# victoriyaforsythe/PyRayHF

Measured on AMD Instinct MI355X. Metric: virtual-height integrals/s (profile x frequency pairs), higher is better.
Workload: dtype f64

## Files before the change

### include/prhf.h

```cpp
#ifndef PRHF_H
#define PRHF_H

#include <stdint.h>

#ifdef __cplusplus
extern "C" {
#endif

#define PRHF_ABI_VERSION 4

#define PRHF_OK        0
#define PRHF_EINVAL   -1
#define PRHF_ENEGDEN  -2
#define PRHF_EPEAK0   -3
#define PRHF_EHIP     -4
#define PRHF_ENOMEM   -5

#define PRHF_MODE_O 0
#define PRHF_MODE_X 1

#define PRHF_FLAG_DEVICE_PTRS 0x1u
#define PRHF_FLAG_ASYNC       0x2u
#define PRHF_FLAG_GRID_STABLE 0x4u
#define PRHF_FLAG_SHARED_FIELD 0x8u
// ... 242 lines not shown
                              const double* scan_elevation_deg, int64_t n_scan, double earth_radius_km, double s_max_km,
                              double rtol, double atol, double max_step_km, double z_ground_km, double top, double left,
                              double right, int32_t renormalize_every, double fill_n, double fill_grad, double fill_mup,
                              double elev_tol_deg, int32_t max_iter, int32_t n_hops, double* out, uint32_t flags);

int prhf_gradient_hop_skip_counters(prhf_ctx* ctx, uint64_t* counters);

int prhf_pair_plan_counters(prhf_ctx* ctx, uint64_t* counters);

int prhf_panel_counters(prhf_ctx* ctx, uint64_t* counters);

int prhf_panel_upper_counters(prhf_ctx* ctx, uint64_t* counters);

int prhf_panel_plan_counters(prhf_ctx* ctx, uint64_t* counters);

int prhf_stream_launches(prhf_ctx* ctx, uint64_t* count);

int prhf_occupancy(prhf_ctx* ctx, int64_t n_alt, int32_t math, int32_t* workgroups_per_cu);

int prhf_sync(prhf_ctx* ctx);

int prhf_last_kernel_ms(prhf_ctx* ctx, double* ms);

int prhf_recent_kernel_ms(prhf_ctx* ctx, double* ms, int32_t capacity, int32_t* n);

#ifdef __cplusplus
}
#endif
#endif
```

### pyrayhf_amd/_native.py

```python

from __future__ import annotations

import ctypes
import os
import threading

_HERE = os.path.dirname(os.path.abspath(__file__))
LIB_PATH = os.environ.get("PRHF_LIB") or os.path.join(_HERE, "libprhf.so")

OK, EINVAL, ENEGDEN, EPEAK0, EHIP, ENOMEM = 0, -1, -2, -3, -4, -5
MODE_O, MODE_X = 0, 1
FLAG_DEVICE_PTRS, FLAG_ASYNC, FLAG_GRID_STABLE, FLAG_SHARED_FIELD = 0x1, 0x2, 0x4, 0x8
MATH_FAITHFUL, MATH_FAST, MATH_AUTO = 0, 1, 2
ABI_VERSION = 4

c_double_p = ctypes.POINTER(ctypes.c_double)


class Segment(ctypes.Structure):
    _fields_ = [("prof_begin", ctypes.c_int64), ("prof_end", ctypes.c_int64),
                ("mode", ctypes.c_int32), ("n_points", ctypes.c_int32),
                ("mult_offset", ctypes.c_int64), ("out_offset", ctypes.c_int64)]


# ... 134 lines not shown
                                   [ctypes.c_int64] + [ctypes.c_void_p, ctypes.c_int64] + [ctypes.c_double] * 9 +
                                   [ctypes.c_int32] + [ctypes.c_double] * 4 +
                                   [ctypes.c_int32, ctypes.c_int32, ctypes.c_void_p, ctypes.c_uint32]),
    "prhf_gradient_hop_muf_f64": (ctypes.c_int, [ctypes.c_void_p, ctypes.c_int32] + [ctypes.c_void_p] * 3 +
                                  [ctypes.c_int64, ctypes.c_int64, ctypes.c_void_p, ctypes.c_void_p, ctypes.c_int32,
                                   ctypes.c_int32] + [ctypes.c_void_p] * 3 +
                                  [ctypes.c_int64, ctypes.c_double, ctypes.c_double, ctypes.c_int32, ctypes.c_void_p,
                                   ctypes.c_int64] + [ctypes.c_double] * 9 + [ctypes.c_int32] + [ctypes.c_double] * 4 +
                                  [ctypes.c_int32, ctypes.c_int32, ctypes.c_void_p, ctypes.c_uint32]),
    "prhf_gradient_skip_counters": (ctypes.c_int, [ctypes.c_void_p, ctypes.POINTER(ctypes.c_uint64)]),
    "prhf_gradient_hop_skip_counters": (ctypes.c_int, [ctypes.c_void_p, ctypes.POINTER(ctypes.c_uint64)]),
    "prhf_pair_plan_counters": (ctypes.c_int, [ctypes.c_void_p, ctypes.POINTER(ctypes.c_uint64)]),
    "prhf_panel_counters": (ctypes.c_int, [ctypes.c_void_p, ctypes.POINTER(ctypes.c_uint64)]),
    "prhf_panel_upper_counters": (ctypes.c_int, [ctypes.c_void_p, ctypes.POINTER(ctypes.c_uint64)]),
    "prhf_panel_plan_counters": (ctypes.c_int, [ctypes.c_void_p, ctypes.POINTER(ctypes.c_uint64)]),
    "prhf_stream_launches": (ctypes.c_int, [ctypes.c_void_p, ctypes.POINTER(ctypes.c_uint64)]),
    "prhf_occupancy": (ctypes.c_int, [ctypes.c_void_p, ctypes.c_int64, ctypes.c_int32,
                                      ctypes.POINTER(ctypes.c_int32)]),
    "prhf_sync": (ctypes.c_int, [ctypes.c_void_p]),
    "prhf_last_kernel_ms": (ctypes.c_int, [ctypes.c_void_p, ctypes.POINTER(ctypes.c_double)]),
    "prhf_recent_kernel_ms": (ctypes.c_int, [ctypes.c_void_p, ctypes.POINTER(ctypes.c_double), ctypes.c_int32,
                                             ctypes.POINTER(ctypes.c_int32)]),
}

_lib = None
_lib_lock = threading.Lock()


def load():
    global _lib
# ... 321 lines not shown
    def panel_counters(self):
        buf = (ctypes.c_uint64 * 2)()
        raise_for(self._lib.prhf_panel_counters(self._h, buf))
        return tuple(int(v) for v in buf)

    def panel_upper_counters(self):
        buf = (ctypes.c_uint64 * 2)()
        raise_for(self._lib.prhf_panel_upper_counters(self._h, buf))
        return tuple(int(v) for v in buf)

    def panel_plan_counters(self):
        buf = (ctypes.c_uint64 * 1)()
        raise_for(self._lib.prhf_panel_plan_counters(self._h, buf))
        return tuple(int(v) for v in buf)

    def stream_launches(self):
        n = ctypes.c_uint64(0)
        raise_for(self._lib.prhf_stream_launches(self._h, ctypes.byref(n)))
        return int(n.value)

    def occupancy(self, n_alt, math):
        n = ctypes.c_int32(0)
        raise_for(self._lib.prhf_occupancy(self._h, int(n_alt), int(math), ctypes.byref(n)))
        return n.value

    def sync(self):
        return self._lib.prhf_sync(self._h)

    def last_kernel_ms(self):
        ms = ctypes.c_double(0.0)
# ... 36 lines not shown
```

### pyrayhf_amd/csrc/prhf_api.cpp

```cpp

#include <hip/hip_runtime_api.h>

#include <algorithm>
#include <cctype>
#include <cmath>
#include <cstdarg>
#include <cstdio>
#include <cstdlib>
#include <cstring>
#include <new>
#include <string>
#include <vector>
#include <xmmintrin.h>

#include "prhf.h"
#include "prhf_kernels.h"
#include "prhf_plan.h"

namespace {

thread_local std::string g_err;

int fail(int code, const char* fmt, ...) {
    char buf[512];
// ... 880 lines not shown
        (e = create_events_untimed(c->slab_up, 3)) != hipSuccess ||
        (e = create_events_untimed(c->slab_done, 3)) != hipSuccess ||
        (e = create_events(c->ring0, prhf_ctx::kTimingRing)) != hipSuccess ||
        (e = create_events(c->ring1, prhf_ctx::kTimingRing)) != hipSuccess ||
        (e = hipMalloc(reinterpret_cast<void**>(&c->d_status), kStatusWords * sizeof(unsigned))) != hipSuccess ||
        (e = hipHostMalloc(reinterpret_cast<void**>(&c->h_status), PRHF_STATUS_WORDS * sizeof(unsigned),
                           hipHostMallocMapped | hipHostMallocCoherent)) != hipSuccess ||
        (e = hipHostGetDevicePointer(reinterpret_cast<void**>(&c->h_status_dev), c->h_status, 0)) != hipSuccess ||
        (e = hipMemset(c->d_status, 0, kStatusWords * sizeof(unsigned))) != hipSuccess ||
        (e = hipHostMalloc(reinterpret_cast<void**>(&c->h_pack), kPackBytes, hipHostMallocMapped | hipHostMallocCoherent)) !=
            hipSuccess ||
        (e = hipHostGetDevicePointer(reinterpret_cast<void**>(&c->h_pack_dev), c->h_pack, 0)) != hipSuccess ||
        (e = hipMalloc(reinterpret_cast<void**>(&c->d_words), 2 * sizeof(unsigned long long))) != hipSuccess ||
        (e = hipHostMalloc(reinterpret_cast<void**>(&c->h_words), 2 * sizeof(unsigned long long),
                           hipHostMallocDefault)) != hipSuccess ||
        (e = hipMalloc(reinterpret_cast<void**>(&c->d_plan_counters), 7 * sizeof(unsigned long long))) != hipSuccess ||
        (e = hipMemset(c->d_plan_counters, 0, 7 * sizeof(unsigned long long))) != hipSuccess ||
        (e = prhf::configure_kernels(staged_lds_bytes(kMaxAlt), kStreamLdsMax)) != hipSuccess) {
        prhf_ctx_destroy(c);
        return fail(PRHF_EHIP, "context setup failed: %s", hipGetErrorString(e));
    }
    c->stream = c->own_stream;
    std::memset(c->h_status, 0, PRHF_STATUS_WORDS * sizeof(unsigned));
#ifdef PRHF_DIAG
    for (const KnobName& k : kKnobNames) {
        std::string env = "PRHF_";
        for (const char* p = k.name; *p; ++p) env += (char)std::toupper((unsigned char)*p);
        if (const char* v = std::getenv(env.c_str())) c->knobs.*(k.field) = std::min(k.hi, std::max(k.lo, std::atof(v)));
    }
#endif
    (void)hipDeviceGetAttribute(&c->cu_count, hipDeviceAttributeMultiprocessorCount, device);
    if (hipDeviceGetAttribute(&c->large_bar, hipDeviceAttributeIsLargeBar, device) != hipSuccess) c->large_bar = 0;
// ... 1967 lines not shown
    counters[0] = w[0] - w[1];
    counters[1] = w[1];
    return PRHF_OK;
}

int prhf_panel_plan_counters(prhf_ctx* c, uint64_t* counters) {
    if (!c || !counters) return fail(PRHF_EINVAL, "null pointer");
    DeviceScope device_scope_(c->device);
    unsigned long long w[1] = {0};
    HIP_TRY(hipStreamSynchronize(c->stream));
    HIP_TRY(hipMemcpy(w, c->d_plan_counters + 6, sizeof w, hipMemcpyDeviceToHost));
    counters[0] = w[0];
    return PRHF_OK;
}

int prhf_stream_launches(prhf_ctx* c, uint64_t* count) {
    if (!c || !count) return fail(PRHF_EINVAL, "null pointer");
    *count = c->stream_launches;
    return PRHF_OK;
}

int prhf_occupancy(prhf_ctx* c, int64_t n_alt, int32_t math, int32_t* workgroups_per_cu) {
    if (!c || !workgroups_per_cu) return fail(PRHF_EINVAL, "null pointer");
    if (n_alt < 1 || n_alt > kMaxAlt) return fail(PRHF_EINVAL, "n_alt out of range");
    ENTER_DEVICE(c->device);
    int n = 0;
    HIP_TRY(prhf::query_occupancy(math, staged_lds_bytes(n_alt), &n));
    *workgroups_per_cu = n;
    return PRHF_OK;
}
// ... 47 lines not shown
```

### pyrayhf_amd/csrc/prhf_kernels.h

```cpp
#ifndef PRHF_KERNELS_H
#define PRHF_KERNELS_H

#include <hip/hip_runtime_api.h>
#include <stddef.h>
#include <stdint.h>

#define PRHF_KMODE_O 0
#define PRHF_KMODE_X 1

#define PRHF_STATUS_NEGDEN 0x1
#define PRHF_STATUS_PEAK0  0x2
#define PRHF_STATUS_BADINDEX 0x4
#define PRHF_STATUS_BADFIELD 0x20
#define PRHF_STATUS_PATHLEN 0x40
#define PRHF_STATUS_WORDS 8
#define PRHF_STATUS_NANINPUT 0x10
#define PRHF_STATUS_BADGROUP 0x8
#define PRHF_STATUS_STALL 0x80

#ifndef PRHF_BLOCK_THREADS
#define PRHF_BLOCK_THREADS 512
#endif
#ifndef PRHF_SHORT_THREADS
#define PRHF_SHORT_THREADS 512
// ... 66 lines not shown
    long long tail_prof;
    int tail_bpp;
    int panel_upper;
    double well_conditioned;
    int lean;
    int prio;
    long long sp_off;
    int strided_lower;
    int panel_lower;
    int panel_nodes;
    int strided_grade;
    int pair_plan;
    int thread_scan;
};

struct KArgs {
    const double* freq;
    const double* den;
    const double* bmag;
    const double* bpsi;
    const double* alt;
    const double* mult;
    const double* pairs;
    const double* ftab;
    double* out;
    double* partial;
    double* altmin;
    unsigned* status;
    unsigned* queue;
    long long n_blocks;
// ... 406 lines not shown
```

### pyrayhf_amd/csrc/prhf_kernels.hip

```cpp

#include <hip/hip_runtime.h>
#include <stdint.h>

#include "prhf_crmath.h"
#include "prhf_kernels.h"

namespace prhf {

namespace {

constexpr double kPlasma = 8.97866275;
constexpr double kGyro = 2.799249247e10;
constexpr double kBackoff = 1e-6;
constexpr double kDegToRad = 0.017453292519943295;
constexpr double kUnmagTol = 1e-12;
constexpr double kLightKmS = 299792.458;
constexpr double kPolyAngle = 3e-4;
constexpr double kQuadAngle = 4e-5;
constexpr double kTrigAngle = 0.05;
constexpr double kLinTol = 1e-10;

struct __attribute__((aligned(16))) Node {
    double alt, off, den, sden, b, sb, u0, u1, u2, u3, psi, spsi;
};
// ... 73 lines not shown
    const int hi = __builtin_amdgcn_update_dpp(__double2hiint(into_lane_0), __double2hiint(v), 0x138, 0xf, 0xf, false);
    return __hiloint2double(hi, lo);
}

__device__ __forceinline__ double uniform(double v) {
    const int lo = __builtin_amdgcn_readfirstlane(__double2loint(v));
    const int hi = __builtin_amdgcn_readfirstlane(__double2hiint(v));
    return __hiloint2double(hi, lo);
}
__device__ __forceinline__ int uniform(int v) { return __builtin_amdgcn_readfirstlane(v); }
constexpr int kStridedLowerBit = 1 << 30;
constexpr int kPanelLowerBit = 1 << 29;
constexpr int kPanelNodes4Bit = 1 << 28;
constexpr int kStridedGradeBit = 1 << 27;
constexpr int kPanelUpperBit = (int)(1u << 31);
constexpr int kPanelFar = 16;
constexpr int kPanelStateShift = 28;
#define PRHF_PANEL_NODES_DECL [[maybe_unused]] static __device__ const double kPanelNodes[8]
#define PRHF_PANEL_PAIRS_DECL static __device__ __attribute__((aligned(16))) const double kPanelPairs[(PRHF_PANEL_N_MAX + 1) * 16]
#include "prhf_panel_table.inc"
#define PRHF_PANEL4_PAIRS_DECL static __device__ __attribute__((aligned(16))) const double kPanel4Pairs[(PRHF_PANEL4_N_MAX + 1) * 8]
#include "prhf_panel4_table.inc"
static_assert(PRHF_PANEL4_N_MAX == PRHF_PANEL_N_MAX, "both tables end at the same piece length");
static_assert(PRHF_PANEL_BLOCK == 64 || PRHF_PANEL_BLOCK == 128, "the weight table ends at 128 points");
static_assert(PRHF_PANEL_BLOCK <= PRHF_PANEL_N_MAX, "a piece holds at most one block");
static_assert(PRHF_PANEL_MIN_SEGMENT >= 1 && (PRHF_PANEL_MIN_SEGMENT & (PRHF_PANEL_MIN_SEGMENT - 1)) == 0,
              "a power of two: the closed form squares its way up");

__device__ __forceinline__ double rsqrt_cubic(double x) {
    const double y = __builtin_amdgcn_rsq(x);
    const double t = x * y;
    const double e = __builtin_fma(-t, y, 1.0);
// ... 819 lines not shown
}
template <class MAt>
__device__ __forceinline__ int panel_first_point(int j, double rkj, double kj, double n1, int i_last, bool& ok, MAt m_at) {
#pragma clang fp contract(fast)
    const int guess = stretch_guess((double)j * rkj, n1);
    const int base = min(max(guess, 0) + 3, i_last) - 3;
    bool hit[4];
#pragma unroll
    for (int q = 0; q < 4; ++q) hit[q] = (int)(m_at(base + q) * kj) >= j;
    ok = j <= 0 || (guess == base && !hit[0] && hit[3]);
    return j <= 0 ? 0 : base + (hit[1] ? 1 : (hit[2] ? 2 : 3));
}
__device__ __forceinline__ int panel_region_end(int lo2) { return ((lo2 + 4) & ~63) & ~(PRHF_PANEL_BLOCK - 1); }
__device__ __forceinline__ int panel_upper_end(int lo0) { return (lo0 + 4) & ~63; }
__device__ __forceinline__ int panel_level(double m, double kj) { return (int)(m * kj); }

template <bool G>
__device__ __forceinline__ TopSegment top_segment(const NodeSpace<G>& nodes_v, int j, double span, double cY) {
#pragma clang fp contract(fast)
    const unsigned nd = __umul24((unsigned)j, (unsigned)sizeof(Node));
    const double o = nodes_v.f64(nd + 8), s = span;
    const double den = nodes_v.f64(nd + 16), sden = nodes_v.f64(nd + 24), b = nodes_v.f64(nd + 32), sb = nodes_v.f64(nd + 40),
                 u0 = nodes_v.f64(nd + 48), u1 = nodes_v.f64(nd + 56), u2 = nodes_v.f64(nd + 64), u3 = nodes_v.f64(nd + 72);
    TopSegment t;
    const SegLinear lin = seg_linear(o, den, sden, b, sb, s, cY);
    t.d0 = lin.d0;  t.d1 = lin.d1;
    t.b0 = lin.b0;  t.b1 = lin.b1;
    t.q0 = u0 + o * (u1 + o * (u2 + o * u3));
    t.q1 = s * (u1 + o * (2.0 * u2 + 3.0 * o * u3));
    t.q2 = (s * s) * (u2 + 3.0 * o * u3);
// ... 253 lines not shown
        }
    };
    constexpr bool STRIDED = TOP && MODE == PRHF_KMODE_X && !CHECK && !G;
    const int i_last_s = last_special;
    bool strided_on = false;
    bool lower_on = false;
    double sc1 = 0.0;
    sp_off = uniform(sp_off);
    const bool lower_req = (sp_off & kStridedLowerBit) != 0;
    const bool panel_req = (sp_off & kPanelLowerBit) != 0;
    const bool nodes4_req = (sp_off & kPanelNodes4Bit) != 0;
    constexpr bool grade_req = GRADE;
    static_assert(!UPPER || (STRIDED && !HINT), "only an instance with the panel block has the upper region");
    sp_off &= ~(kStridedLowerBit | kPanelLowerBit | kPanelNodes4Bit | kStridedGradeBit | kPanelUpperBit);
    constexpr int kUpperKept = 16, kUpperRegion = 8;
    int panel_state = 0;
    asm volatile("" : "+v"(panel_state));
    if (STRIDED && sp_off > 0 && n_seg > 0 && first == 0 && last_special >= 0 && end >= PRHF_TOP3_MIN_POINTS) {
        if constexpr (UPPER) {
            if (plan_panel) {
                typedef unsigned int u32x2 __attribute__((ext_vector_type(2)));
                const u32x2 vc = __builtin_amdgcn_raw_buffer_load_b64(rsrc, 0, sp_off * (int)sizeof(double2) + 8, 0);
                __builtin_memcpy(&sc1, &vc, sizeof sc1);
                strided_on = true;
                lower_on = lower_req;
            } else {
                const u32x4 vh = __builtin_amdgcn_raw_buffer_load_b128(rsrc, 0, sp_off * (int)sizeof(double2), 0);
                double2 gh;
                __builtin_memcpy(&gh, &vh, sizeof gh);
                const int hw = uniform((int)vh.x);
                strided_on = (hw & 1) == 0;
// ... 124 lines not shown
        int S_R = 0, E_R = 0, n_R = 0;
        const double n1 = (double)i_last_s, rkj = uniform(1.0 / kj);
        int j_b0 = seg_j[2];
        auto index_of = [&](double m) {
            const double A = __builtin_fma(1.0 - m, 22025.465794806718, 1.0);
            if (!(A > 0.0)) return 1e9;
            const double ln_a = (double)__builtin_amdgcn_logf((float)A) * 0.6931471805599453;
            return fmin(fmax(__builtin_fma(-ln_a, n1 * 0.1, n1), -1e9), 1e9);
        };
        auto x_of = [&](int j) { return index_of((double)j * rkj); };
        if (lower && panel_req && end < 65536) {
            bool panel_ok = false;
            int S_P = 0;
            constexpr int B = PRHF_PANEL_BLOCK, kLogB = B == 128 ? 7 : 6;
            const double c0 = 1.0 / 22025.465794806718;
            panel_state = 2;
            asm volatile("" : "+v"(panel_state));
            auto first_point = [&](int j, bool& ok) {
                return panel_first_point(j, rkj, kj, n1, i_last_s, ok, [&](int i) {
                    typedef unsigned int u32x2 __attribute__((ext_vector_type(2)));
                    const u32x2 v = __builtin_amdgcn_raw_buffer_load_b64(rsrc, (unsigned)i * (unsigned)sizeof(double2), 0, 0);
                    double mq;
                    __builtin_memcpy(&mq, &v, sizeof mq);
                    return mq;
                });
            };
            auto region_end = [&]() { return panel_region_end(seg_lo[2]); };
            constexpr bool REC = UPPER && PLANNABLE;
            unsigned pw3 = 0u, pw5 = 0u;
            if constexpr (REC) {
                const unsigned plan_s = (unsigned)uniform((int)plan_v);
// ... 42 lines not shown
                bool fail = false;
                int j_0 = j_s, left = j_e - j_s + 1;
                int j_e_lo = j_e, e_v = E_lo, s_v = S_P;
                if constexpr (UPPER) {
                    asm volatile("" : "+v"(j_e_lo), "+v"(s_v));
                    int up;
                    if (from_rec) {
                        up = (int)((pw3 >> 10) & 3u);
                    } else {
                        const u32x4 vu = __builtin_amdgcn_raw_buffer_load_b128(rsrc, 0, (upper_end() - 1) * (int)sizeof(double2), 0);
                        double2 gu;
                        __builtin_memcpy(&gu, &vu, sizeof gu);
                        up = uniform(panel_level(gu.x, kj)) - (seg_j[0] - 1);
                    }
                    if (up == 0 || up == 1) {
                        panel_state = 2 | kUpperRegion;
                        left = seg_j[0] + up - j_s;
                        e_v = upper_end();
                    } else {
                        panel_state = 2 | kUpperKept;
                    }
                    asm volatile("" : "+v"(e_v));
                }
#pragma unroll 1
                while (left > 0) {
                    int E_P = E_lo, S_L = S_P;
                    if constexpr (UPPER) {
                        asm volatile("" : "+v"(j_e_lo), "+v"(e_v), "+v"(s_v));
                        E_P = e_v;
                        S_L = s_v;
                    }
                    const bool live = lane < left;
                    const int j_g = live ? j_0 + lane : j_0;
                    bool ok;
                    const int fq = first_point(j_g, ok);
                    const int p = live ? max(fq, S_L) : E_P;
                    const int p_next = __shfl_down(p, 1);
                    const int n = live && lane < 63 ? max(min(p_next, E_P) - p, 0) : 0;
                    const int k = (n + B - 1) >> kLogB;
                    int L = n;
                    if (__any(k > 1)) {
                        int q = (int)((float)n * __builtin_amdgcn_rcpf((float)max(k, 1)));
                        q += q * k < n ? 1 : 0;
                        q -= (q - 1) * k >= n ? 1 : 0;
                        L = k > 1 ? q : n;
                    }
                    const unsigned nd = __umul24((unsigned)j_g, (unsigned)sizeof(Node));
                    const double o = nodes_v.f64(nd + 8), den = nodes_v.f64(nd + 16), sden = nodes_v.f64(nd + 24),
                                 bf = nodes_v.f64(nd + 32), sb = nodes_v.f64(nd + 40);
                    const double sl = cX * (sden * span) + r2 * (cYs * (sb * span));
                    const double gap = 1.0 - cX * (den + sden * o) - r2 * (cYs * (bf + sb * o));
                    const double m_hi = (double)(j_g + 1) * rkj;
                    const double g_lo = gap - sl * ((double)j_g * rkj), g_hi = gap - sl * m_hi;
                    const bool big = n > 8;
                    const bool levels = g_lo >= 1e-6 && g_hi >= 1e-6;
                    bool clear = levels;
                    const bool far = sl > 0.0 && (n1 * 0.1) * g_hi >= (double)(4 * B + 2) * (sl * ((1.0 - m_hi) + c0));
                    const int k_chk = big && clear && !far && __builtin_fabs(sl) > 1e-300 ? k : 0;
                    if (__any(k_chk > 0)) {
                        const double i_sing = index_of(gap / sl);
                        for (int i = 0; __ballot(i < k_chk) != 0ull; ++i) {
                            const int n_i = min(L, n - i * L);
                            const double c = (double)(p + i * L) + 0.5 * (double)(n_i - 1);
                            if (i < k_chk && n_i > 8)
                                clear = clear && __builtin_fabs(i_sing - c) >= fmax(32.0, 4.0 * (double)n_i);
                        }
                    }
                    int lvl = 0;
                    if (nodes4_req) {
                        bool open = n > 0;
                        for (int t = 0;; ++t) {
                            if (open) {
                                const int n_s = (L + (1 << t) - 1) >> t;
                                const double kk = (double)(kPanelFar * n_s + 2);
                                const double i_far = sl < 0.0 ? ((double)p + 0.5 * (double)((L >> t) - 1)) - kk
                                                              : ((double)(p + n - 1) - 0.5 * (double)(n_s - 1)) + kk;
                                const double e_far = (double)__builtin_amdgcn_exp2f((float)(i_far * (s10 * 1.4426950408889634)));
                                lvl = t;
                                open = !(n_s <= 4 || (levels && (1.0 + c0) * sl - gap <= sl * ((1.0 + c0) * e_far)));
                            }
                            if (__ballot(open) == 0ull) break;
                        }
                    }
                    const int cnt = n > 0 ? k << lvl : 0;
                    if constexpr (UPPER) {
                        int bad_v = (live && !ok) || (big && !clear) || cnt > 128 ? 1 : 0;
                        fail = __ballot(bad_v != 0) != 0ull;
                        if (fail) {
                            asm volatile("" : "+v"(bad_v));
                            if (!upper_now() || __ballot(bad_v != 0 && j_g < seg_j[0] - 3) != 0ull) break;
                            fail = false;
                            if (left <= 63) {
                                panel_state = 2 | kUpperKept;
                                e_v = region_end();
                                left = uniform(j_e_lo) - j_0 + 1;
                                continue;
                            }
                        }
                    } else {
                        fail = __ballot((live && !ok) || (big && !clear) || cnt > 128) != 0ull;
                        if (fail) break;
                    }
                    int total = min(63, left), n_take = total;
                    if constexpr (UPPER) {
                        if (left > 63 && upper_now()) total = n_take = min(total, seg_j[0] - 3 - j_0);
                    }
                    unsigned lst_a = n > 0 && (!UPPER || lane < total) ? (unsigned)p | ((unsigned)n << 16) : 0u, lst_b = 0u;
                    if (__ballot(cnt != (live && lane < 63 ? 1 : 0)) != 0ull) {
                        int incl = cnt;
                        incl += __builtin_amdgcn_update_dpp(0, incl, 0x111, 0xf, 0xf, false);
                        incl += __builtin_amdgcn_update_dpp(0, incl, 0x112, 0xf, 0xf, false);
                        incl += __builtin_amdgcn_update_dpp(0, incl, 0x114, 0xf, 0xf, false);
                        incl += __builtin_amdgcn_update_dpp(0, incl, 0x118, 0xf, 0xf, false);
                        incl += __builtin_amdgcn_update_dpp(0, incl, 0x142, 0xa, 0xf, false);
                        incl += __builtin_amdgcn_update_dpp(0, incl, 0x143, 0xc, 0xf, false);
                        n_take = __builtin_popcountll(__ballot((UPPER ? lane < total : live && lane < 63) && incl <= 128));
                        total = __builtin_amdgcn_readlane(incl, n_take - 1);
// ... 73 lines not shown
                                eval(eb);
                                break;
                            }
                            fetch(k0, ea);
                            eval(eb);
                        }
                    }
                }
                panel_ok = !fail;
                if constexpr (UPPER) S_P = uniform(s_v);
                if (!panel_ok) accm = 0.0;
                g0 = grid_at(first);
            }
            if constexpr (UPPER) {
                const int flags = uniform(panel_state);
                panel_state = !panel_ok ? 2 : ((flags & kUpperRegion) != 0 ? 3 : 4);
                asm volatile("" : "+v"(panel_state));
                if (panel_ok) {
                    S_R = S_P;
                    E_R = (flags & kUpperRegion) != 0 ? upper_end() : region_end();
                    n_R = -1;
                }
            } else if (panel_ok) {
                panel_state = 1;
                asm volatile("" : "+v"(panel_state));
                S_R = S_P;
                E_R = region_end();
                n_R = -1;
            }
        }
        if (lower && n_R >= 0) {
// ... 86 lines not shown
                    idx = (j_whole + (t0 + lane - 32 * n_R)) << 3;
                    coef = 8.0;
                }
                const u32x4 vm = __builtin_amdgcn_raw_buffer_load_b128(rsrc, (unsigned)idx * (unsigned)sizeof(double2), 0, 0);
                double2 gm;
                __builtin_memcpy(&gm, &vm, sizeof gm);
                gm.y = coef * (sc1 * ((1.0 - gm.x) + c0));
                accm = lean_step<MODE, false, POLY, HINT, G>(gm, span, a0v, kj, cX, hcY2, accm, wc, viol, nodes_v, cur);
            }
            }
            first = E_R;
            g0 = grid_at(first);
        }
    }
    if (TOP) {
        const int sidx_0 = UPPER && uniform(panel_state) == 3 ? 0 : n_seg - 1;
#pragma unroll 1
        for (int sidx = sidx_0; sidx >= 0 && !(CHECK && viol); --sidx) {
            const int lo_b = sidx == 0 ? seg_lo[0] : (sidx == 1 ? seg_lo[1] : seg_lo[2]);
            const int begin_s = (lo_b + 63) & ~63;
            const int end_s = sidx == 0 ? whole_end : ((sidx == 1 ? seg_lo[0] : seg_lo[1]) & ~63);
            const int j_s = seg_j[0] - sidx;
            run_indexed(begin_s);
            if (!(CHECK && viol)) {
                top = top_segment(nodes_v, j_s, span, cYs);
                if (STRIDED && strided_on) {
                    const int lo_s = sidx == 0 ? seg_lo[0] : (sidx == 1 ? seg_lo[1] : seg_lo[2]);
                    const int q_s = sidx == 0 ? i_last_s - 1 : (sidx == 1 ? seg_lo[0] - 1 : seg_lo[1] - 1);
                    strided_run(lo_s, q_s, begin_s, sidx);
                }
                run_top(end_s);
// ... 14 lines not shown
        } else {
            if (!live) g = make_double2(HINT ? uniform(g0.x) : 0.0, 0.0);
            a1 = lean_step<MODE, CHECK, POLY, HINT, G>(g, span, a0v, kj, cX, hcY2, accm, wc, viol, nodes_v, cur);
        }
        if (!(CHECK && viol)) {
            accm = a1;
            first = end;
        } else {
            const int L = __ffsll((long long)viol) - 1;
            if (lane < L) accm = a1;
            first += L;
        }
    }
    LeanResult r;
    r.acc = accm * span;
    r.first = first | (panel_state << kPanelStateShift);
    return r;
}

template <int MODE, bool CHECK, int POLY, bool HINT, bool TOP, bool G, bool GRADE, bool UPPER>
__device__ __attribute__((noinline)) LeanResult lean_loop_region(typename NodeArg<G>::type nodes_arg, unsigned hint_lds,
                                                                 const double2* __restrict__ pairs, int first, int end,
                                                                 int last_special, double span, double a0, double kj,
                                                                 double cX, double cY2, double well_conditioned, int sp_off) {
    return lean_loop_body<MODE, CHECK, POLY, HINT, TOP, G, GRADE, UPPER>(nodes_arg, hint_lds, pairs, first, end, last_special,
                                                                          span, a0, kj, cX, cY2, well_conditioned, sp_off);
}
template <int MODE, bool CHECK, int POLY, bool HINT, bool TOP, bool G, bool GRADE>
__device__ __attribute__((noinline)) LeanResult lean_loop_instance(typename NodeArg<G>::type nodes_arg, unsigned hint_lds,
                                                                   const double2* __restrict__ pairs, int first, int end,
                                                                   int last_special, double span, double a0, double kj,
// ... 75 lines not shown
            else if (lean_end - first >= PRHF_TOP_MIN_POINTS && i0 == 0 && to_grid_end) r = PRHF_LEAN_POLY(false, true);
            else r = PRHF_LEAN_POLY(false, false);
#undef PRHF_LEAN_POLY
#undef PRHF_LEAN
            if (uniform((int)__any(!(__builtin_fabs(r.acc) <= 1.7976931348623157e308)))) {
                acc = 0.0;
                first = uniform(i0);
#ifdef PRHF_MARK_FALLBACK
                acc = 1e6;
#endif
            } else {
                acc = r.acc;
                first = uniform(r.first) & ((1 << kPanelStateShift) - 1);
            }
            panel_state = uniform(r.first) >> kPanelStateShift;
        }
    }
    const int n_iter = uniform((i1 - first + 63) >> 6);
    int i = i1 - (n_iter << 6) + lane;
    auto grid = [&](int idx) { return mult[idx < first ? first : (idx < last ? idx : last)]; };
    double m0 = 0.0, m1 = 0.0;
    if (n_iter > 0) {
        m0 = grid(i);
        m1 = grid(i + 1);
    }
    for (int it = 0; it < n_iter; ++it) {
        const int inext = i + 64;
        const double n0 = grid(inext);
        const double n1 = grid(inext + 1);
        const bool active = i >= first;
// ... 469 lines not shown
                                          const PlanRoom& room) {
    constexpr int W = THREADS / 64;
    const int lane = threadIdx.x & 63;
    const double* keep = kept_scalars<THREADS>(red);
    const double wc = uniform(sg.well_conditioned);
    const int F = uniform((int)a.n_freq);
    const int C = uniform(sg.chunks);
    const int T = info.n_cand >= 0 ? info.n_cand : F * C;
    const double* mult = a.mult + sg.mult_off;
    const double2* pairs = (a.pairs && sg.lean) ? reinterpret_cast<const double2*>(a.pairs) + sg.mult_off : nullptr;
    const int sp_off = (pairs && sg.sp_off > 0)
                           ? uniform((int)(sg.sp_off - sg.mult_off) | (sg.strided_lower ? kStridedLowerBit : 0) |
                                     (sg.strided_lower && sg.panel_lower ? kPanelLowerBit : 0) |
                                     (sg.strided_lower && sg.panel_lower && sg.panel_nodes == 4 ? kPanelNodes4Bit : 0) |
                                     (!G && sg.strided_lower && sg.panel_lower && sg.panel_upper ? kPanelUpperBit : 0) |
                                     (sg.strided_grade ? kStridedGradeBit : 0)) : 0;
    const long long pair_base = prof_local * F;
    const int first_item = block_in_prof * W, round_items = blocks_per_prof * W;
    static_assert(11 * W + 8 <= PRHF_RED_DOUBLES, "reduction scratch too small");
    const int S = uniform(sg.slots), wave = threadIdx.x >> 6;
    const bool local = S > 0;
    double* part = red + 10 * W + 8;
    if (local && lane == 0) part[wave] = 0.0;
    int pulled = 0;
    int panel_cnt = 0;
    auto next_item = [&]() {
        const int u = uniform(atomicAdd(item_next, 1)) >> 6;
        pulled = u;
        return uniform((u / W) * round_items + first_item + (u % W));
    };
    int t = local ? uniform(block_in_prof * W + wave) : next_item();
    const int t_end = local ? uniform(min(F * S, t + 1)) : T;
    for (; t < t_end; t = local ? t_end : next_item()) {
        int f = t, c = 0;
        if (local) {
            f = t / S;
            c = t % S;
            if (c >= C) break;
        } else if (info.n_cand >= 0) {
            f = uniform((int)cand[t]);
// ... 17 lines not shown
            } else if (reflects) {
                const int i0 = c * sg.chunk_len;
                const int i1 = min(sg.n_points, i0 + sg.chunk_len);
                if (info.unmag)
                    result = integrate_chunk<MODE, TIER, true, G>(nodes, hint, info, mult, pairs, sg.n_points, i0, i1,
                                                               pf.f_hz, pf.f2, pf.cX, pf.cY2, h, lane, wc, sp_off, plan_lds, panel);
                else
                    result = integrate_chunk<MODE, TIER, false, G>(nodes, hint, info, mult, pairs, sg.n_points, i0,
                                                                i1, pf.f_hz, pf.f2, pf.cX, pf.cY2, h, lane, wc, sp_off, plan_lds, panel);
            } else if (info.K == 1) {
                result = (c == C - 1) ? one_level_term<MODE, TIER>(nodes, info, pf, sg.well_conditioned) : 0.0;
                reflects = true;
            }
        }
        if constexpr (MODE == PRHF_KMODE_X && TIER == 1 && !G) {
            panel_cnt += panel == 2 ? 0x10000 : (panel != 0 ? 1 : 0);
            if (panel == 4 && lane == 0 && a.plan_counters) atomicAdd(&a.plan_counters[5], 1ull);
        }
        if (lane == 0) {
            if (local) {
                part[wave] = reflects ? result : qnan();
            } else if (C == 1) {
                const double vh = (reflects && result != 0.0) ? result + keep[kKeepAltMin] : qnan();
                a.out[sg.out_off + pair_base + f] = vh;
            } else {
                a.partial[sg.partial_off + (pair_base + f) * C + c] = reflects ? result : qnan();
            }
        }
    }
    if constexpr (MODE == PRHF_KMODE_X && TIER == 1 && !G) {
        if (lane == 0 && a.plan_counters) {
            if (panel_cnt & 0xffff) atomicAdd(&a.plan_counters[2], (unsigned long long)(panel_cnt & 0xffff));
            if (panel_cnt >> 16) atomicAdd(&a.plan_counters[3], (unsigned long long)(panel_cnt >> 16));
            if (sg.panel_upper && (panel_cnt & 0xffff)) atomicAdd(&a.plan_counters[4], (unsigned long long)(panel_cnt & 0xffff));
        }
    }
    if (local) {
        __syncthreads();
        const int item = block_in_prof * W + wave;
        const int f = item / S;
        if (f < F && item % S == 0 && lane == 0) {
            double sum = 0.0;
            for (int cc = 0; cc < C; ++cc) sum = sum + part[wave + cc];
            a.out[sg.out_off + pair_base + f] = (sum == sum && sum != 0.0) ? sum + keep[kKeepAltMin] : qnan();
        }
    }
}

}

// ... 923 lines not shown
```

### pyrayhf_amd/csrc/prhf_plan.h

```cpp

#ifndef PRHF_PLAN_H
#define PRHF_PLAN_H

#include <algorithm>
#include <cmath>
#include <cstdint>
#include <cstdio>
#include <cstring>

#include "prhf.h"
#include "prhf_kernels.h"

namespace {

struct Knobs {
    double target_waves = 4096;
    double lean_min_points = 65;
    double well_conditioned = 1e-5;
    double thread_scan_min = 0.0;
    double no_candidates = 0;
    double persistent = 1;
    double tail_rounds = 1.0;
    double tail_bpp = 4;
    double split_min_points = 1024;
// ... 6 lines not shown
    double timing = 0;
    double trim_lds = 1;
    double short_compact = 1;
    double short_prio = 4;
    double short_order = 1;
    double short_lanes = 0;
    double host_slabs = 3;
    double local_chunks = 1;
    double tall_lean = 1;
    double snell_table = 4;
    double strided_top = 1;
    double strided_lower = 1;
    double panel_lower = 1;
    double panel_nodes = 4;
    double panel_upper = 1;
    double strided_grade = 1;
    double pair_plan = 1;
    double pair_plan_cap = 0;
    double stream_blocks = 1;
    double stream_grid = 0;
};
struct KnobName {
    const char* name;
    double Knobs::*field;
    double lo, hi;
};
const KnobName kKnobNames[] = {
    {"target_waves", &Knobs::target_waves, 64, 1e9},
    {"lean_min_points", &Knobs::lean_min_points, 2, 1e9},
    {"well_conditioned", &Knobs::well_conditioned, 0, 1},
// ... 12 lines not shown
    {"direct_upload", &Knobs::direct_upload, 0, 1},
    {"timing", &Knobs::timing, 0, 1},
    {"trim_lds", &Knobs::trim_lds, 0, 1},
    {"short_compact", &Knobs::short_compact, 0, 1},
    {"short_prio", &Knobs::short_prio, 0, 7},
    {"host_slabs", &Knobs::host_slabs, 1, 3},
    {"short_order", &Knobs::short_order, 0, 1},
    {"short_lanes", &Knobs::short_lanes, 0, 16},
    {"snell_table", &Knobs::snell_table, 0, 1e9},
    {"tall_lean", &Knobs::tall_lean, 0, 1},
    {"strided_top", &Knobs::strided_top, 0, 1},
    {"strided_lower", &Knobs::strided_lower, 0, 1},
    {"panel_lower", &Knobs::panel_lower, 0, 1},
    {"panel_nodes", &Knobs::panel_nodes, 4, 8},
    {"panel_upper", &Knobs::panel_upper, 0, 1},
    {"strided_grade", &Knobs::strided_grade, 0, 1},
    {"pair_plan", &Knobs::pair_plan, 0, 1},
    {"pair_plan_cap", &Knobs::pair_plan_cap, 0, 1024},
    {"stream_blocks", &Knobs::stream_blocks, 0, 2},
    {"stream_grid", &Knobs::stream_grid, 0, 65536},
};
constexpr int kWavesPerBlock = PRHF_BLOCK_THREADS / 64;

inline void plan_slice(prhf::SegDev& s, long long n_freq, long long wg_slots, const Knobs& kn) {
    const long long kTargetWaves = (long long)kn.target_waves;
    const bool kSplitFewProfiles = kn.split_few_profiles != 0;
    const long long kSplitMinPoints = (long long)kn.split_min_points;
    const double kTailRounds = kn.tail_rounds;
    const int kTailBpp = (int)kn.tail_bpp;
    const long long P = s.prof_end - s.prof_begin;
// ... 345 lines not shown
            int p = 0;
            while (p < pieces.n && !(pieces.mult_off[p] == s.mult_off && pieces.n_points[p] == s.n_points)) ++p;
            if (p == pieces.n) {
                const long long len = prhf::strided_piece_entries(s.n_points);
                if ((pl.table_entries + len) * 16 >= 0x7fffffffLL) continue;
                pieces.mult_off[p] = s.mult_off;
                pieces.n_points[p] = s.n_points;
                pieces.sp_off[p] = pl.table_entries;
                pl.table_entries += len;
                ++pieces.n;
            }
            s.sp_off = pieces.sp_off[p];
            s.strided_lower = kn.strided_lower != 0;
            s.panel_lower = s.strided_lower && kn.panel_lower != 0;
            s.panel_nodes = s.panel_lower && kn.panel_nodes == 4 ? 4 : 8;
            s.panel_upper = s.panel_lower && kn.panel_upper != 0;
            s.strided_grade = kn.strided_grade != 0;
            s.pair_plan = slice_plans_pairs(s, tall, n_freq, lds_levels, kn) ? 1 : 0;
            pl.any_plan = pl.any_plan || s.pair_plan != 0;
        }
    }
    pl.stream = false;
    pl.stream_grid = 0;
    pl.stream_lds_bytes = 0;
    pl.stream_blocks = 0;
    pl.stream_tail_bpp = 0;
    pl.stream_tail_prof = 0;
    if (kn.stream_blocks != 0 && kPersistent && !tall && pl.n_segs == 1 && pl.o.n_segs == 0 && pl.x.n_segs == 0 && pl.blocks > 0 &&
        (pl.queue || kn.stream_blocks == 2) && 2 * pl.lds_bytes <= kLdsFull) {
        Knobs with_plans = kn;
        with_plans.pair_plan = 1;
// ... 115 lines not shown
```

Measured before the change: 392.1 million.

## Add quick bound test to skip exact panel-level checks in upper region

Adds a cheap per-wave sufficient-condition test (panel_run_quick) in the upper panel region of the X-mode tier-1 kernel. When every lane passes it, the kernel skips loading the node's five values and the exact clearance and level refinement and goes straight to the listed path. A new panel_quick knob, on by default, enables it, and per-block slotted counters are added to track quick versus exact passes. The counter bookkeeping adds atomics and more packed state bits, and the bound must stay conservative to keep accuracy.

```diff
diff --git a/include/prhf.h b/include/prhf.h
--- a/include/prhf.h
+++ b/include/prhf.h
@@ -280,6 +280,8 @@
 
 int prhf_panel_plan_counters(prhf_ctx* ctx, uint64_t* counters);
 
+int prhf_panel_quick_counters(prhf_ctx* ctx, uint64_t* counters);
+
 int prhf_stream_launches(prhf_ctx* ctx, uint64_t* count);
 
 int prhf_occupancy(prhf_ctx* ctx, int64_t n_alt, int32_t math, int32_t* workgroups_per_cu);
diff --git a/pyrayhf_amd/_native.py b/pyrayhf_amd/_native.py
--- a/pyrayhf_amd/_native.py
+++ b/pyrayhf_amd/_native.py
@@ -172,6 +172,7 @@
     "prhf_panel_counters": (ctypes.c_int, [ctypes.c_void_p, ctypes.POINTER(ctypes.c_uint64)]),
     "prhf_panel_upper_counters": (ctypes.c_int, [ctypes.c_void_p, ctypes.POINTER(ctypes.c_uint64)]),
     "prhf_panel_plan_counters": (ctypes.c_int, [ctypes.c_void_p, ctypes.POINTER(ctypes.c_uint64)]),
+    "prhf_panel_quick_counters": (ctypes.c_int, [ctypes.c_void_p, ctypes.POINTER(ctypes.c_uint64)]),
     "prhf_stream_launches": (ctypes.c_int, [ctypes.c_void_p, ctypes.POINTER(ctypes.c_uint64)]),
     "prhf_occupancy": (ctypes.c_int, [ctypes.c_void_p, ctypes.c_int64, ctypes.c_int32,
                                       ctypes.POINTER(ctypes.c_int32)]),
@@ -523,6 +524,11 @@
         raise_for(self._lib.prhf_panel_plan_counters(self._h, buf))
         return tuple(int(v) for v in buf)
 
+    def panel_quick_counters(self):
+        buf = (ctypes.c_uint64 * 2)()
+        raise_for(self._lib.prhf_panel_quick_counters(self._h, buf))
+        return tuple(int(v) for v in buf)
+
     def stream_launches(self):
         n = ctypes.c_uint64(0)
         raise_for(self._lib.prhf_stream_launches(self._h, ctypes.byref(n)))
diff --git a/pyrayhf_amd/csrc/prhf_api.cpp b/pyrayhf_amd/csrc/prhf_api.cpp
--- a/pyrayhf_amd/csrc/prhf_api.cpp
+++ b/pyrayhf_amd/csrc/prhf_api.cpp
@@ -918,8 +918,8 @@
         (e = hipMalloc(reinterpret_cast<void**>(&c->d_words), 2 * sizeof(unsigned long long))) != hipSuccess ||
         (e = hipHostMalloc(reinterpret_cast<void**>(&c->h_words), 2 * sizeof(unsigned long long),
                            hipHostMallocDefault)) != hipSuccess ||
-        (e = hipMalloc(reinterpret_cast<void**>(&c->d_plan_counters), 7 * sizeof(unsigned long long))) != hipSuccess ||
-        (e = hipMemset(c->d_plan_counters, 0, 7 * sizeof(unsigned long long))) != hipSuccess ||
+        (e = hipMalloc(reinterpret_cast<void**>(&c->d_plan_counters), prhf::kPlanCounterWords * sizeof(unsigned long long))) != hipSuccess ||
+        (e = hipMemset(c->d_plan_counters, 0, prhf::kPlanCounterWords * sizeof(unsigned long long))) != hipSuccess ||
         (e = prhf::configure_kernels(staged_lds_bytes(kMaxAlt), kStreamLdsMax)) != hipSuccess) {
         prhf_ctx_destroy(c);
         return fail(PRHF_EHIP, "context setup failed: %s", hipGetErrorString(e));
@@ -2917,6 +2917,20 @@
     return PRHF_OK;
 }
 
+int prhf_panel_quick_counters(prhf_ctx* c, uint64_t* counters) {
+    if (!c || !counters) return fail(PRHF_EINVAL, "null pointer");
+    DeviceScope device_scope_(c->device);
+    unsigned long long w[prhf::kQuickSlots * prhf::kQuickSlotWords];
+    HIP_TRY(hipStreamSynchronize(c->stream));
+    HIP_TRY(hipMemcpy(w, c->d_plan_counters + prhf::kQuickSlotBase, sizeof w, hipMemcpyDeviceToHost));
+    counters[0] = counters[1] = 0;
+    for (int s = 0; s < prhf::kQuickSlots; ++s) {
+        counters[0] += w[s * prhf::kQuickSlotWords];
+        counters[1] += w[s * prhf::kQuickSlotWords + 1];
+    }
+    return PRHF_OK;
+}
+
 int prhf_stream_launches(prhf_ctx* c, uint64_t* count) {
     if (!c || !count) return fail(PRHF_EINVAL, "null pointer");
     *count = c->stream_launches;
diff --git a/pyrayhf_amd/csrc/prhf_kernels.h b/pyrayhf_amd/csrc/prhf_kernels.h
--- a/pyrayhf_amd/csrc/prhf_kernels.h
+++ b/pyrayhf_amd/csrc/prhf_kernels.h
@@ -104,6 +104,9 @@
     int thread_scan;
 };
 
+constexpr int kQuickSlots = 64, kQuickSlotWords = 8, kQuickSlotBase = 8;
+constexpr int kPlanCounterWords = kQuickSlotBase + kQuickSlots * kQuickSlotWords;
+
 struct KArgs {
     const double* freq;
     const double* den;
diff --git a/pyrayhf_amd/csrc/prhf_kernels.hip b/pyrayhf_amd/csrc/prhf_kernels.hip
--- a/pyrayhf_amd/csrc/prhf_kernels.hip
+++ b/pyrayhf_amd/csrc/prhf_kernels.hip
@@ -111,8 +111,10 @@
 constexpr int kPanelNodes4Bit = 1 << 28;
 constexpr int kStridedGradeBit = 1 << 27;
 constexpr int kPanelUpperBit = (int)(1u << 31);
+constexpr int kPanelQuickBit = 1 << 26;
 constexpr int kPanelFar = 16;
 constexpr int kPanelStateShift = 28;
+constexpr int kPanelQuickShift = 16;
 #define PRHF_PANEL_NODES_DECL [[maybe_unused]] static __device__ const double kPanelNodes[8]
 #define PRHF_PANEL_PAIRS_DECL static __device__ __attribute__((aligned(16))) const double kPanelPairs[(PRHF_PANEL_N_MAX + 1) * 16]
 #include "prhf_panel_table.inc"
@@ -962,6 +964,16 @@
 __device__ __forceinline__ int panel_region_end(int lo2) { return ((lo2 + 4) & ~63) & ~(PRHF_PANEL_BLOCK - 1); }
 __device__ __forceinline__ int panel_upper_end(int lo0) { return (lo0 + 4) & ~63; }
 __device__ __forceinline__ int panel_level(double m, double kj) { return (int)(m * kj); }
+__device__ __forceinline__ bool panel_run_quick(double g_j, double g_n, double kj, double m_lo, double m_hi, double n1, int L) {
+#pragma clang fp contract(fast)
+    const double c0 = 1.0 / 22025.465794806718;
+    const double sl = (g_j - g_n) * kj;
+    const double D = L <= 4 ? 0.0 : (double)(kPanelFar * L + 10);
+    const bool up = sl >= 0.0;
+    const double lhs = (n1 * 0.1) * (up ? g_n : g_j);
+    const double rhs = up ? D * (sl * ((1.0 - m_hi) + c0)) : D * (g_j - sl * ((1.0 - m_lo) + c0));
+    return g_j >= 1e-3 && g_n >= 1e-3 && lhs >= rhs;
+}
 
 template <bool G>
 __device__ __forceinline__ TopSegment top_segment(const NodeSpace<G>& nodes_v, int j, double span, double cY) {
@@ -1245,7 +1257,12 @@
     static_assert(!UPPER || (STRIDED && !HINT), "only an instance with the panel block has the upper region");
     sp_off &= ~(kStridedLowerBit | kPanelLowerBit | kPanelNodes4Bit | kStridedGradeBit | kPanelUpperBit);
     constexpr int kUpperKept = 16, kUpperRegion = 8;
+    constexpr int kQuickOn = 32, kQuickPass = 1 << 8, kExactPass = 1 << 20;
     int panel_state = 0;
+    if constexpr (UPPER) {
+        panel_state = (sp_off & kPanelQuickBit) != 0 ? kQuickOn : 0;
+        sp_off &= ~kPanelQuickBit;
+    }
     asm volatile("" : "+v"(panel_state));
     if (STRIDED && sp_off > 0 && n_seg > 0 && first == 0 && last_special >= 0 && end >= PRHF_TOP3_MIN_POINTS) {
         if constexpr (UPPER) {
@@ -1400,7 +1417,8 @@
             int S_P = 0;
             constexpr int B = PRHF_PANEL_BLOCK, kLogB = B == 128 ? 7 : 6;
             const double c0 = 1.0 / 22025.465794806718;
-            panel_state = 2;
+            if constexpr (UPPER) panel_state = (panel_state & kQuickOn) | 2;
+            else panel_state = 2;
             asm volatile("" : "+v"(panel_state));
             auto first_point = [&](int j, bool& ok) {
                 return panel_first_point(j, rkj, kj, n1, i_last_s, ok, [&](int i) {
@@ -1473,11 +1491,11 @@
                         up = uniform(panel_level(gu.x, kj)) - (seg_j[0] - 1);
                     }
                     if (up == 0 || up == 1) {
-                        panel_state = 2 | kUpperRegion;
+                        panel_state |= kUpperRegion;
                         left = seg_j[0] + up - j_s;
                         e_v = upper_end();
                     } else {
-                        panel_state = 2 | kUpperKept;
+                        panel_state |= kUpperKept;
                     }
                     asm volatile("" : "+v"(e_v));
                 }
@@ -1504,6 +1522,30 @@
                         q -= (q - 1) * k >= n ? 1 : 0;
                         L = k > 1 ? q : n;
                     }
+                    bool quick = false;
+                    if constexpr (UPPER) {
+                        asm volatile("" : "+v"(panel_state));
+                        if ((uniform(panel_state) & kQuickOn) != 0) {
+                            const unsigned nq = __umul24((unsigned)(j_0 + min(lane, left)), (unsigned)sizeof(Node));
+                            const double g_j = 1.0 - cX * nodes_v.f64(nq + 16) - r2 * (cYs * nodes_v.f64(nq + 32));
+                            const double g_n = __shfl_down(g_j, 1);
+                            const bool pass = !live || (ok && k <= 128 &&
+                                                        (n == 0 || panel_run_quick(g_j, g_n, kj, (double)j_g * rkj,
+                                                                                   (double)(j_g + 1) * rkj, n1, L)));
+                            quick = __ballot(!pass) == 0ull;
+                        }
+                    }
+                    int lvl = 0, cnt = 0;
+                    if constexpr (UPPER) {
+                        if (quick) {
+                            cnt = n > 0 ? k : 0;
+                            fail = false;
+                            panel_state += kQuickPass;
+                            goto listed;
+                        }
+                        panel_state += kExactPass;
+                    }
+                    {
                     const unsigned nd = __umul24((unsigned)j_g, (unsigned)sizeof(Node));
                     const double o = nodes_v.f64(nd + 8), den = nodes_v.f64(nd + 16), sden = nodes_v.f64(nd + 24),
                                  bf = nodes_v.f64(nd + 32), sb = nodes_v.f64(nd + 40);
@@ -1525,7 +1567,6 @@
                                 clear = clear && __builtin_fabs(i_sing - c) >= fmax(32.0, 4.0 * (double)n_i);
                         }
                     }
-                    int lvl = 0;
                     if (nodes4_req) {
                         bool open = n > 0;
                         for (int t = 0;; ++t) {
@@ -1541,7 +1582,7 @@
                             if (__ballot(open) == 0ull) break;
                         }
                     }
-                    const int cnt = n > 0 ? k << lvl : 0;
+                    cnt = n > 0 ? k << lvl : 0;
                     if constexpr (UPPER) {
                         int bad_v = (live && !ok) || (big && !clear) || cnt > 128 ? 1 : 0;
                         fail = __ballot(bad_v != 0) != 0ull;
@@ -1550,7 +1591,7 @@
                             if (!upper_now() || __ballot(bad_v != 0 && j_g < seg_j[0] - 3) != 0ull) break;
                             fail = false;
                             if (left <= 63) {
-                                panel_state = 2 | kUpperKept;
+                                panel_state = (panel_state & ~kUpperRegion) | kUpperKept;
                                 e_v = region_end();
                                 left = uniform(j_e_lo) - j_0 + 1;
                                 continue;
@@ -1560,6 +1601,8 @@
                         fail = __ballot((live && !ok) || (big && !clear) || cnt > 128) != 0ull;
                         if (fail) break;
                     }
+                    }
+                listed: __attribute__((unused));
                     int total = min(63, left), n_take = total;
                     if constexpr (UPPER) {
                         if (left > 63 && upper_now()) total = n_take = min(total, seg_j[0] - 3 - j_0);
@@ -1663,7 +1706,7 @@
             }
             if constexpr (UPPER) {
                 const int flags = uniform(panel_state);
-                panel_state = !panel_ok ? 2 : ((flags & kUpperRegion) != 0 ? 3 : 4);
+                panel_state = (flags & ~(kQuickPass - 1)) | (!panel_ok ? 2 : ((flags & kUpperRegion) != 0 ? 3 : 4));
                 asm volatile("" : "+v"(panel_state));
                 if (panel_ok) {
                     S_R = S_P;
@@ -1780,7 +1823,7 @@
         }
     }
     if (TOP) {
-        const int sidx_0 = UPPER && uniform(panel_state) == 3 ? 0 : n_seg - 1;
+        const int sidx_0 = UPPER && (uniform(panel_state) & 7) == 3 ? 0 : n_seg - 1;
 #pragma unroll 1
         for (int sidx = sidx_0; sidx >= 0 && !(CHECK && viol); --sidx) {
             const int lo_b = sidx == 0 ? seg_lo[0] : (sidx == 1 ? seg_lo[1] : seg_lo[2]);
@@ -1825,7 +1868,14 @@
     }
     LeanResult r;
     r.acc = accm * span;
-    r.first = first | (panel_state << kPanelStateShift);
+    if constexpr (UPPER) {
+        const unsigned ps = (unsigned)uniform(panel_state);
+        const unsigned n_quick = min((ps >> 8) & 0xfffu, 63u), n_exact = min(ps >> 20, 63u);
+        r.first = first | (int)((ps & 7u) << kPanelStateShift) | (int)(n_quick << kPanelQuickShift) |
+                  (int)(n_exact << (kPanelQuickShift + 6));
+    } else {
+        r.first = first | (panel_state << kPanelStateShift);
+    }
     return r;
 }
 
@@ -1931,6 +1981,12 @@
                 first = uniform(r.first) & ((1 << kPanelStateShift) - 1);
             }
             panel_state = uniform(r.first) >> kPanelStateShift;
+            if constexpr (MODE == PRHF_KMODE_X && TIER == 1 && !G) {
+                if (panel_state != 0) {
+                    panel_state |= ((uniform(r.first) >> kPanelQuickShift) & 0xfff) << 4;
+                    first &= 0xffff;
+                }
+            }
         }
     }
     const int n_iter = uniform((i1 - first + 63) >> 6);
@@ -2430,6 +2486,8 @@
                                      (sg.strided_lower && sg.panel_lower ? kPanelLowerBit : 0) |
                                      (sg.strided_lower && sg.panel_lower && sg.panel_nodes == 4 ? kPanelNodes4Bit : 0) |
                                      (!G && sg.strided_lower && sg.panel_lower && sg.panel_upper ? kPanelUpperBit : 0) |
+                                     (!G && info.uniform && sg.strided_lower && sg.panel_lower && (sg.panel_upper & 2)
+                                          ? kPanelQuickBit : 0) |
                                      (sg.strided_grade ? kStridedGradeBit : 0)) : 0;
     const long long pair_base = prof_local * F;
     const int first_item = block_in_prof * W, round_items = blocks_per_prof * W;
@@ -2439,7 +2497,20 @@
     double* part = red + 10 * W + 8;
     if (local && lane == 0) part[wave] = 0.0;
     int pulled = 0;
-    int panel_cnt = 0;
+    unsigned panel_cnt = 0u;
+    auto flush_panel_cnt = [&]() {
+        if (lane == 0 && a.plan_counters) {
+            const unsigned took = panel_cnt & 0xffu, fell = (panel_cnt >> 8) & 0xffu;
+            const unsigned n_quick = (panel_cnt >> 16) & 0xffu, n_exact = panel_cnt >> 24;
+            if (took) atomicAdd(&a.plan_counters[2], (unsigned long long)took);
+            if (fell) atomicAdd(&a.plan_counters[3], (unsigned long long)fell);
+            if (sg.panel_upper && took) atomicAdd(&a.plan_counters[4], (unsigned long long)took);
+            unsigned long long* slot = a.plan_counters + kQuickSlotBase + (blockIdx.x & (kQuickSlots - 1)) * kQuickSlotWords;
+            if (n_quick) atomicAdd(slot, (unsigned long long)n_quick);
+            if (n_exact) atomicAdd(slot + 1, (unsigned long long)n_exact);
+        }
+        panel_cnt = 0u;
+    };
     auto next_item = [&]() {
         const int u = uniform(atomicAdd(item_next, 1)) >> 6;
         pulled = u;
@@ -2487,8 +2558,11 @@
             }
         }
         if constexpr (MODE == PRHF_KMODE_X && TIER == 1 && !G) {
-            panel_cnt += panel == 2 ? 0x10000 : (panel != 0 ? 1 : 0);
-            if (panel == 4 && lane == 0 && a.plan_counters) atomicAdd(&a.plan_counters[5], 1ull);
+            const int state = panel & 15;
+            panel_cnt += (state == 2 ? 0x100u : (state != 0 ? 1u : 0u)) | (((unsigned)panel >> 4) & 63u) << 16 |
+                         (((unsigned)panel >> 10) & 63u) << 24;
+            if ((panel_cnt & 0x80808080u) != 0u) flush_panel_cnt();
+            if (state == 4 && lane == 0 && a.plan_counters) atomicAdd(&a.plan_counters[5], 1ull);
         }
         if (lane == 0) {
             if (local) {
@@ -2502,11 +2576,7 @@
         }
     }
     if constexpr (MODE == PRHF_KMODE_X && TIER == 1 && !G) {
-        if (lane == 0 && a.plan_counters) {
-            if (panel_cnt & 0xffff) atomicAdd(&a.plan_counters[2], (unsigned long long)(panel_cnt & 0xffff));
-            if (panel_cnt >> 16) atomicAdd(&a.plan_counters[3], (unsigned long long)(panel_cnt >> 16));
-            if (sg.panel_upper && (panel_cnt & 0xffff)) atomicAdd(&a.plan_counters[4], (unsigned long long)(panel_cnt & 0xffff));
-        }
+        if (panel_cnt != 0u) flush_panel_cnt();
     }
     if (local) {
         __syncthreads();
diff --git a/pyrayhf_amd/csrc/prhf_plan.h b/pyrayhf_amd/csrc/prhf_plan.h
--- a/pyrayhf_amd/csrc/prhf_plan.h
+++ b/pyrayhf_amd/csrc/prhf_plan.h
@@ -44,6 +44,7 @@
     double panel_lower = 1;
     double panel_nodes = 4;
     double panel_upper = 1;
+    double panel_quick = 1;
     double strided_grade = 1;
     double pair_plan = 1;
     double pair_plan_cap = 0;
@@ -86,6 +87,7 @@
     {"panel_lower", &Knobs::panel_lower, 0, 1},
     {"panel_nodes", &Knobs::panel_nodes, 4, 8},
     {"panel_upper", &Knobs::panel_upper, 0, 1},
+    {"panel_quick", &Knobs::panel_quick, 0, 1},
     {"strided_grade", &Knobs::strided_grade, 0, 1},
     {"pair_plan", &Knobs::pair_plan, 0, 1},
     {"pair_plan_cap", &Knobs::pair_plan_cap, 0, 1024},
@@ -461,7 +463,8 @@
             s.strided_lower = kn.strided_lower != 0;
             s.panel_lower = s.strided_lower && kn.panel_lower != 0;
             s.panel_nodes = s.panel_lower && kn.panel_nodes == 4 ? 4 : 8;
-            s.panel_upper = s.panel_lower && kn.panel_upper != 0;
+            s.panel_upper = s.panel_lower && kn.panel_upper != 0 && s.sp_off - s.mult_off < (1LL << 26)
+                                ? 1 | (kn.panel_quick != 0 ? 2 : 0) : 0;
             s.strided_grade = kn.strided_grade != 0;
             s.pair_plan = slice_plans_pairs(s, tall, n_freq, lds_levels, kn) ? 1 : 0;
             pl.any_plan = pl.any_plan || s.pair_plan != 0;
```

After: 398.3 million, median of 6. 1.6% higher.
